# chenc10/distributed_TensorFlow_models

Measured on AMD Instinct MI355X. Metric: images/sec (whole node) ResNet-50 224×224 bf16 at 1/2/4/8 MI355X, higher is better.
Workload: dtype bf16; 1 GPU; model=resnet_v1_50, global_batch=256, per_gpu_batch=256, image_size=224, parallelism=dp1, device=cuda, grad_allreduce_dtype=fp32, deterministic=True, optimizer=momentum-sgd+wd

## Files before the change

csrc/kernels/conv_igemm.hip:

```cpp
#include "common.h"
#include <cstdio>

namespace dtm {


struct ConvNTArgs {
  const bf16_t* x;
  const bf16_t* w;
  bf16_t* y;
  float* stats;
  const float* bias;
  const float* in_scale;
  const float* in_shift;
  uint32_t x_bytes, w_bytes;
  int N, Hin, Win, C, K, R, S, P, Q;
  int stride, pad_h, pad_w;
  int Hv, Wv;
  int M;
  int Kg;
  int relu;
  FastDiv fd_PQ, fd_Q;
  const bf16_t* add_src;
  int add_stride;
  int add_H, add_W;
// ... 37 lines not shown
#undef DTM_GRP_LOAD
  }
  return t % gxy;
}

__device__ __forceinline__ void out_nhw(const ConvNTArgs& a, int m, int& n, int& h, int& w) {
  if (a.sp_tw) {
    const uint32_t t = (uint32_t)m >> 7, l = (uint32_t)m & 127u;
    const uint32_t nn = fdiv(t, a.fd_sp_img), rem = t - nn * (a.sp_th * a.sp_tw);
    const uint32_t th = fdiv(rem, a.fd_sp_tw), tw = rem - th * a.sp_tw;
    n = (int)nn;
    h = (int)(th * 8u + (l >> 4));
    w = (int)(tw * 16u + (l & 15u));
    return;
  }
  const uint32_t nn = fdiv((uint32_t)m, a.fd_PQ), rem = m - nn * (a.P * a.Q);
  const uint32_t i = fdiv(rem, a.fd_Q), j = rem - i * a.Q;
  n = (int)nn;
  h = (int)i * a.ostr + a.oa;
  w = (int)j * a.ostr + a.ob;
}
__device__ __forceinline__ int out_row(const ConvNTArgs& a, int m) {
  if (a.ostr == 1 && !a.sp_tw) return m;
  int n, h, w;
  out_nhw(a, m, n, h, w);
  return (n * a.OH + h) * a.OW + w;
}

__device__ __forceinline__ bool out_valid(const ConvNTArgs& a, int m) {
  if (!a.sp_tw) return true;
  int n, h, w;
  out_nhw(a, m, n, h, w);
  return h < a.P && w < a.Q;
}

template <bool RAWB>
__device__ __forceinline__ void epi_barrier() {
  if constexpr (RAWB) {
    asm volatile("s_waitcnt lgkmcnt(0)" ::: "memory");
    __builtin_amdgcn_s_barrier();
  } else {
    __syncthreads();
  }
}

template <int PT, int CT, bool RAWB, bool EXACT, bool SACC, int NT, bool SIDE = true, bool PRE = false, bool SPL = false,
          int EG = 4>
__device__ __forceinline__ void conv_nt_epi_tail(const ConvNTArgs& a, char* smem, int p0, int c0, int by,
                                                 float* ssum, float* ssq, const char* pre = nullptr,
                                                 const float* pre_ss = nullptr, float* aacc = nullptr) {
  constexpr int OROW = CT * 2 + 16;
  const int tid = threadIdx.x;
  epi_barrier<RAWB>();
  constexpr int CPR = CT / 8;
  constexpr int NIT = PT * CPR / NT;
  static_assert(NT % CPR == 0 && (PT * CPR) % NT == 0, "staged-store mapping");
  const int chn = tid % CPR;
  const int kc = c0 + chn * 8;
  const bool act = SIDE && a.act_x != nullptr;
  const bool bstats = !SACC && a.stats != nullptr;
  float sc[8], sh[8], sgx[8], sg[8];
#pragma unroll
  for (int e = 0; e < 8; ++e) { sc[e] = 1.f; sh[e] = 0.f; sgx[e] = 0.f; sg[e] = 0.f; }
  const bool amask = act && a.act_mask != nullptr;
  float sgr[8];
#pragma unroll
  for (int e = 0; e < 8; ++e) sgr[e] = 0.f;
  if (act && !amask && kc < a.K) {
#pragma unroll
    for (int e = 0; e < 8; ++e) {
      sc[e] = PRE ? pre_ss[chn * 8 + e] : a.act_ss[kc + e];
      sh[e] = PRE ? pre_ss[CT + chn * 8 + e] : a.act_ss[a.K + kc + e];
    }
  }
  constexpr int GRP = NIT < EG ? NIT : EG;
  static_assert(NIT % GRP == 0, "epilogue row groups");
  const bool side = SIDE && (a.add_src != nullptr || act);
#pragma unroll
  for (int g0 = 0; g0 < NIT; g0 += GRP) {
    uint4 pa[GRP], px[GRP], pr[GRP];
    uint32_t pm[GRP];
    bool ph[GRP];
#pragma unroll
    for (int j = 0; j < GRP; ++j) {
      pa[j] = px[j] = pr[j] = make_uint4(0, 0, 0, 0);
      pm[j] = 0u;
      ph[j] = false;
    }
    if (PRE && side) {
#pragma unroll
      for (int j = 0; j < GRP; ++j) {
        if (a.add_src) {
          pa[j] = *(const uint4*)(pre + (size_t)(g0 + j) * NT * 16 + tid * 16);
          ph[j] = true;
        }
        if (act) px[j] = *(const uint4*)(pre + (size_t)(NIT + g0 + j) * NT * 16 + tid * 16);
      }
    } else if (side) {
#pragma unroll
      for (int j = 0; j < GRP; ++j) {
        const int row = ((g0 + j) * NT + tid) / CPR;
        const int m = p0 + row;
        if (m < a.M && kc < a.K && out_valid(a, m)) {
          const size_t o = (size_t)out_row(a, m) * a.K + kc;
          if (a.add_src) {
            const bf16_t* src = a.add_src + o;
// ... 887 lines not shown
#pragma unroll
      for (int ii = 0; ii < 2; ++ii) {
        const int row = ni * 128 + wq * 32 + ii * 16 + fr;
        const short8 v = *(const short8*)(s + 2 * HALF + row * 128 + (((ks * 4 + fk) ^ (row & 7)) << 4));
        if (ni == 0) Wa[ks][ii] = v;
        else Wb[ks][ii] = v;
      }
  };
  auto mma = [&](int ni, int mi) {
#pragma unroll
    for (int ks = 0; ks < 2; ++ks)
#pragma unroll
      for (int ii = 0; ii < 2; ++ii)
#pragma unroll
        for (int jj = 0; jj < 4; ++jj)
          acc[ni][ii][mi][jj] = __builtin_amdgcn_mfma_f32_16x16x32_bf16(ni == 0 ? Wa[ks][ii] : Wb[ks][ii], P[ks][jj],
                                                                        acc[ni][ii][mi][jj], 0, 0, 0);
  };
  pp_mainloop(smem, BUF, nk, grp, issue, rd_p, rd_w, mma);
  __syncthreads();

#pragma unroll
  for (int ni = 0; ni < 2; ++ni)
#pragma unroll
    for (int ii = 0; ii < 2; ++ii) {
      const int kloc = ni * 128 + wq * 32 + ii * 16 + fk * 4;
      float bia[4] = {0.f, 0.f, 0.f, 0.f};
      if (a.bias && c0 + kloc < a.K) {
#pragma unroll
        for (int r = 0; r < 4; ++r) bia[r] = a.bias[c0 + kloc + r];
      }
#pragma unroll
      for (int mi = 0; mi < 2; ++mi)
#pragma unroll
        for (int jj = 0; jj < 4; ++jj) {
          const int mloc = mi * 128 + grp * 64 + jj * 16 + fr;
          float v[4];
#pragma unroll
          for (int r = 0; r < 4; ++r) {
            v[r] = acc[ni][ii][mi][jj][r] + bia[r];
            if (a.relu) v[r] = fmaxf(v[r], 0.f);
          }
          *(uint2*)(smem + mloc * OROW + kloc * 2) = make_uint2(pack2bf(v[0], v[1]), pack2bf(v[2], v[3]));
        }
    }
  conv_nt_epi_tail<PT, CT, false, false, false, 512, true, false, SPL>(a, smem, p0, c0, by, nullptr, nullptr);
}

template <int CT>
__device__ __forceinline__ void worker_row(float* red, const float* lo, const float* hi, float* row, int c0, int K) {
  constexpr int CPR = CT / 8, RPT = 256 / CPR;
  const int tid = threadIdx.x;
  __syncthreads();
#pragma unroll
  for (int e = 0; e < 8; ++e) { red[tid * 16 + e] = lo[e]; red[tid * 16 + 8 + e] = hi[e]; }
  __syncthreads();
  for (int h = RPT / 2; h >= 1; h >>= 1) {
    if (tid < h * CPR) {
#pragma unroll
      for (int e = 0; e < 16; ++e) red[tid * 16 + e] += red[(tid + h * CPR) * 16 + e];
    }
    __syncthreads();
  }
  const int kc = c0 + tid * 8;
  if (tid < CPR && kc < K) {
#pragma unroll
    for (int e = 0; e < 8; ++e) { row[kc + e] = red[tid * 16 + e]; row[K + kc + e] = red[tid * 16 + 8 + e]; }
  }
}

__device__ __forceinline__ void glds16(const void* gptr, const void* lds) {
  const uint32_t l = __builtin_amdgcn_readfirstlane((uint32_t)(uintptr_t)(const __attribute__((address_space(3))) void*)lds);
  asm volatile("s_mov_b32 m0, %1\n\ts_nop 0\n\tglobal_load_lds_dwordx4 %0, off" ::"v"(gptr), "s"(l) : "memory", "m0");
}

template <int PT, int CT, int NKT, bool PRO, bool STEM = false, int NBUF = 2, bool SIDE = true>
__global__ __launch_bounds__(256) void conv1x1_stream_kernel(ConvNTArgs a, int ntiles) {
  constexpr int WP = PT / 2, WC = CT / 2;
  constexpr int TP = WP / 16, TC = WC / 16;
  constexpr int AI = PT / 32, WI = CT / 32;
  constexpr int ABUF = NKT * PT * 128;
  constexpr int WBUF = NKT * CT * 128;
  constexpr int OROW = CT * 2 + 16;
  constexpr int STG = PT * OROW > 16384 ? PT * OROW : 16384;
  constexpr int NIT = PT * (CT / 8) / 256;
  constexpr int MAXC = 512;
  constexpr int OFF_A = WBUF, OFF_S = WBUF + NBUF * ABUF, OFF_P = OFF_S + STG;
  constexpr int NDMA = NKT * AI;
  static_assert(NBUF == 2 || NBUF == 3, "ring depth");
  static_assert(2 * NIT + NDMA <= 63, "vmcnt range");
  __shared__ __attribute__((aligned(16))) char smem[OFF_P + (PRO ? MAXC * 8 : 0)];
  typedef __attribute__((address_space(1))) const void gvoid;
  typedef __attribute__((address_space(3))) void lvoid;
  static_assert(NIT >= 1 && NIT <= 15, "vmcnt lower bound");

  const int tid = threadIdx.x, lane = tid & 63, wave = tid >> 6;
  const int nb = gridDim.x * gridDim.y;
  const int bid = xcd_remap(blockIdx.y * gridDim.x + blockIdx.x, nb);
  const int bx = bid % gridDim.x, by0 = bid / gridDim.x;
  const int c0 = bx * CT;
  const int lr = lane >> 3;
  const int ch = (lane & 7) ^ lr;
  const char* xg = (const char*)a.x;
  const char* wg = (const char*)a.w;
  const char* zg = (const char*)a.zero;
  float* s_scale = (float*)(smem + OFF_P);
  float* s_shift = s_scale + MAXC;
  if constexpr (PRO) {
    for (int c = tid; c < a.C; c += 256) { s_scale[c] = a.in_scale[c]; s_shift[c] = a.in_shift[c]; }
  }
#pragma unroll
  for (int kt = 0; kt < NKT; ++kt) {
#pragma unroll
    for (int j = 0; j < WI; ++j) {
      const int row = c0 + 8 * (wave + 4 * j) + lr;
      const int k = kt * 64 + ch * 8;
      const bool v = (row < a.K) & (k < a.Kg);
      const char* src = wg + (size_t)(uint32_t)((row * a.Kg + k) * 2);
      __builtin_amdgcn_global_load_lds((gvoid*)(v ? src : zg), (lvoid*)(smem + kt * CT * 128 + (wave + 4 * j) * 1024),
                                       16, 0, 0);
    }
  }
  const char* srcs[NKT * AI];
  auto issue = [&](int t, int buf) {
    char* base = smem + OFF_A + buf * ABUF;
    uint32_t pix[AI];
    if constexpr (STEM) {
#pragma unroll
      for (int j = 0; j < AI; ++j) {
        const int m = t * PT + 8 * (wave + 4 * j) + lr;
        const uint32_t mm = m < a.M ? (uint32_t)m : 0u;
        const uint32_t n = fdiv(mm, a.fd_PQ), rem = mm - n * (a.P * a.Q);
        const uint32_t p = fdiv(rem, a.fd_Q), q = rem - p * a.Q;
        pix[j] = ((n * a.Hin + p * a.stride) * a.Win + q * a.stride) * 8u;
      }
    }
#pragma unroll
    for (int kt = 0; kt < NKT; ++kt) {
      const int k = kt * 64 + ch * 8;
#pragma unroll
      for (int j = 0; j < AI; ++j) {
        const int m = t * PT + 8 * (wave + 4 * j) + lr;
        const bool v = (m < a.M) & (k < a.Kg);
        const char* src = STEM ? xg + (size_t)(pix[j] + (uint32_t)((k >> 5) * a.Win * 8 + (k & 31) * 2))
                               : xg + (size_t)(uint32_t)(m * a.pix_bytes + k * 2);
        srcs[kt * AI + j] = v ? src : zg;
        glds16(srcs[kt * AI + j], base + kt * PT * 128 + (wave + 4 * j) * 1024);
      }
    }
  };
  auto transform = [&](int t, int buf) {
    char* base = smem + OFF_A + buf * ABUF;
#pragma unroll
    for (int kt = 0; kt < NKT; ++kt) {
      const int k = kt * 64 + ch * 8;
      if (k < a.Kg) {
        const float4 s0 = *(const float4*)(s_scale + k), s1 = *(const float4*)(s_scale + k + 4);
        const float4 h0 = *(const float4*)(s_shift + k), h1 = *(const float4*)(s_shift + k + 4);
        const float sc[8] = {s0.x, s0.y, s0.z, s0.w, s1.x, s1.y, s1.z, s1.w};
        const float sh[8] = {h0.x, h0.y, h0.z, h0.w, h1.x, h1.y, h1.z, h1.w};
#pragma unroll
        for (int j = 0; j < AI; ++j) {
          const int m = t * PT + 8 * (wave + 4 * j) + lr;
          if (m < a.M) {
            uint4* pp = (uint4*)(base + kt * PT * 128 + (wave + 4 * j) * 1024 + lane * 16);
            const uint4 q = *pp;
            uint32_t u[4] = {q.x, q.y, q.z, q.w};
#pragma unroll
            for (int e = 0; e < 4; ++e) {
              const float lo = fmaxf(fmaf(lo_bf(u[e]), sc[2 * e], sh[2 * e]), 0.f);
              const float hi = fmaxf(fmaf(hi_bf(u[e]), sc[2 * e + 1], sh[2 * e + 1]), 0.f);
              u[e] = pack2bf(lo, hi);
            }
            *pp = make_uint4(u[0], u[1], u[2], u[3]);
          }
        }
      }
    }
  };

  const int wp = wave % 2, wc = wave / 2;
  const int fr = lane & 15, fk = lane >> 4;
  float ssum[8], ssq[8], aacc[24];
#pragma unroll
  for (int e = 0; e < 8; ++e) { ssum[e] = 0.f; ssq[e] = 0.f; }
#pragma unroll
  for (int e = 0; e < 24; ++e) aacc[e] = 0.f;
  int t = by0;
  const int gy = gridDim.y;
  if (t < ntiles) issue(t, 0);
  if (NBUF == 3 && t + gy < ntiles) issue(t + gy, 1);
  asm volatile("s_waitcnt vmcnt(0)" ::: "memory");
  __syncthreads();
  int buf = 0;
  for (int it = 0; t < ntiles; ++it, t += gy) {
    if constexpr (NBUF == 2) {
      if (it > 0) asm volatile("s_waitcnt vmcnt(%0)" ::"n"(NIT) : "memory");
    } else if (it >= 2) {
      if (t + gy < ntiles) asm volatile("s_waitcnt vmcnt(%0)" ::"n"(2 * NIT + NDMA) : "memory");
      else asm volatile("s_waitcnt vmcnt(%0)" ::"n"(2 * NIT) : "memory");
    }
    if constexpr (PRO) transform(t, buf);
    asm volatile("s_waitcnt lgkmcnt(0)" ::: "memory");
    __builtin_amdgcn_s_barrier();
    if constexpr (NBUF == 2) {
      if (t + gy < ntiles) issue(t + gy, buf ^ 1);
    } else {
      if (t + 2 * gy < ntiles) issue(t + 2 * gy, buf == 0 ? 2 : buf - 1);
    }
    f32x4 acc[TC][TP];
#pragma unroll
    for (int i = 0; i < TC; ++i)
#pragma unroll
      for (int j = 0; j < TP; ++j) acc[i][j] = (f32x4){0.f, 0.f, 0.f, 0.f};
    const char* abase = smem + OFF_A + buf * ABUF;
#pragma unroll
    for (int kt = 0; kt < NKT; ++kt) {
#pragma unroll
      for (int ks = 0; ks < 2; ++ks) {
        short8 bf[TP], af[TC];
        const int chn = ks * 4 + fk;
#pragma unroll
        for (int j = 0; j < TP; ++j) {
          const int row = wp * WP + j * 16 + fr;
          bf[j] = *(const short8*)(abase + kt * PT * 128 + row * 128 + ((chn ^ (row & 7)) << 4));
        }
#pragma unroll
        for (int i = 0; i < TC; ++i) {
          const int row = wc * WC + i * 16 + fr;
          af[i] = *(const short8*)(smem + kt * CT * 128 + row * 128 + ((chn ^ (row & 7)) << 4));
        }
#pragma unroll
        for (int i = 0; i < TC; ++i)
#pragma unroll
          for (int j = 0; j < TP; ++j)
            acc[i][j] = __builtin_amdgcn_mfma_f32_16x16x32_bf16(af[i], bf[j], acc[i][j], 0, 0, 0);
      }
    }
    conv_nt_epilogue<PT, CT, WP, WC, 1, true, true, true, true, 256, SIDE>(a, acc, smem + OFF_S, t * PT, c0, t, ssum,
                                                                           ssq, nullptr, nullptr, aacc);
#pragma unroll
    for (int i = 0; i < NKT * AI; ++i) asm volatile("" ::"v"(srcs[i]));
    buf = buf + 1 == NBUF ? 0 : buf + 1;
  }
  asm volatile("s_waitcnt vmcnt(0)" ::: "memory");
  if (a.stats) worker_row<CT>((float*)(smem + OFF_S), ssum, ssq, a.stats + (size_t)by0 * (2 * a.K), c0, a.K);
  if (SIDE && a.act_x && a.act_sums) {
    const int rw = a.act_r ? 4 : 2;
    float* row = a.act_sums + (size_t)by0 * (rw * a.K);
    worker_row<CT>((float*)(smem + OFF_S), aacc, aacc + 8, row, c0, a.K);
    if (a.act_r) worker_row<CT>((float*)(smem + OFF_S), aacc + 16, aacc + 8, row + 2 * a.K, c0, a.K);
  }
}

template <int CIN>
__device__ __forceinline__ int dsw(int p, int c) {
  return CIN == 64 ? (c ^ ((p >> 1) & 7)) : (c ^ ((p >> 2) & 3));
}

template <int CIN, int CT, bool SIDE>
__global__ __launch_bounds__(256) void conv3x3_direct_kernel(ConvNTArgs a, int ntiles) {
  constexpr int TH = 8, TW = 16, PT = TH * TW, HH = TH + 2, HW = TW + 2;
  constexpr int CPP = CIN / 8;
  constexpr int HCH = HH * HW * CPP;
  constexpr int NDMA = (HCH + 255) / 256;
  constexpr int OROW = CT * 2 + 16;
  constexpr int HDMA = NDMA * 256 * 16;
  constexpr int HBUF = HDMA > PT * OROW ? HDMA : PT * OROW;
  static_assert(3 * HBUF >= 256 * 16 * 4, "worker_row's reduction table fits in the ring");
  constexpr int WBUF = 9 * CT * CIN * 2;
  constexpr int NIT = PT * (CT / 8) / 256;
  constexpr int TC = CT / 16, TP = 2;
  constexpr int SD = SIDE ? 2 * NIT : 0;
  constexpr int SBUF = SIDE ? 2 * NIT * 4096 + 2 * CT * 4 : 0;
  static_assert(2 * NIT + SD + NDMA <= 63, "vmcnt range");
  __shared__ __attribute__((aligned(16))) char smem[WBUF + 3 * HBUF + SBUF];
  char* sside = smem + WBUF + 3 * HBUF;
  float* s_ss = (float*)(sside + 2 * NIT * 4096);

  const int tid = threadIdx.x, lane = tid & 63, wave = tid >> 6;
  const int nb = gridDim.x * gridDim.y;
  const int bid = xcd_remap(blockIdx.y * gridDim.x + blockIdx.x, nb);
  const int bx = bid % gridDim.x, by0 = bid / gridDim.x;
  const int c0 = bx * CT;
  const char* xg = (const char*)a.x;
  const char* zg = (const char*)a.zero;
  const int tiles_w = a.sp_tw, tiles_img = a.sp_th * a.sp_tw;

  if constexpr (SIDE) {
    for (int j = tid; j < 2 * CT; j += 256) {
      const int ch = j % CT, k = c0 + ch;
      s_ss[j] = (a.act_x && k < a.K) ? a.act_ss[(j / CT) * a.K + k] : (j < CT ? 1.f : 0.f);
// ... 988 lines not shown
  const int n = flip_tiles(f);
  for (int t = blockIdx.x; t < n; t += gridDim.x) flip_tile(f, t, lds);
}

}

using namespace dtm;

struct ConvDesc {
  int N, H, W, C, K, R, S, P, Q, stride, pad_h, pad_w;
  int pix_bytes;
  int dec;
};

static const bf16_t* zero_chunk() {
  static void* z = nullptr;
  if (!z) {
    if (hipMalloc(&z, 4096) != hipSuccess) return nullptr;
    hipMemset(z, 0, 4096);
    hipDeviceSynchronize();
  }
  return (const bf16_t*)z;
}
const void* dtm_zero_chunk() { return zero_chunk(); }

template <int PT, int CT, int NWP, int NS, int UD, bool SPL = false, int NTH = 512>
static void launch_w8(const ConvNTArgs& a, hipStream_t st) {
  dim3 grid((a.K + CT - 1) / CT, (a.M + PT - 1) / PT, a.ngrp > 1 ? a.ngrp : 1);
  hipLaunchKernelGGL((conv_nt_w8_kernel<PT, CT, NWP, NS, UD, SPL, NTH>), grid, dim3(NTH), 0, st, a);
}

template <int UD, bool SPL = false>
static void launch_pp(const ConvNTArgs& a, hipStream_t st) {
  dim3 grid((a.K + 255) / 256, (a.M + 255) / 256, a.ngrp > 1 ? a.ngrp : 1);
  hipLaunchKernelGGL((conv_nt_pp_kernel<UD, SPL>), grid, dim3(512), 0, st, a);
}

template <int PT, int CT, int NS, int UD, int NWP = 2, bool SPL = false>
static void launch_pipe(const ConvNTArgs& a, hipStream_t st) {
  dim3 grid((a.K + CT - 1) / CT, (a.M + PT - 1) / PT, a.ngrp > 1 ? a.ngrp : 1);
  if (SPL) hipLaunchKernelGGL((conv_nt_pipe_kernel<PT, CT, NS, UD, false, NWP, true>), grid, dim3(256), 0, st, a);
  else if (a.in_scale) hipLaunchKernelGGL((conv_nt_pipe_kernel<PT, CT, NS, UD, true, NWP>), grid, dim3(256), 0, st, a);
  else hipLaunchKernelGGL((conv_nt_pipe_kernel<PT, CT, NS, UD, false, NWP>), grid, dim3(256), 0, st, a);
}

static int device_cus() { return dtm_compute_cus(); }

static bf16_t* dump_chunk() {
  static void* z = nullptr;
  if (!z && hipMalloc(&z, 4096) != hipSuccess) return nullptr;
  return (bf16_t*)z;
}

template <int PT, int CT, int NKT, bool PRO, bool STEM = false, int NBUF = 2, bool SIDE = true>
static int stream_workers_k(const ConvNTArgs& a) {
  static int occ = 0;
  if (!occ) {
    if (hipOccupancyMaxActiveBlocksPerMultiprocessor(&occ, conv1x1_stream_kernel<PT, CT, NKT, PRO, STEM, NBUF, SIDE>,
                                                     256, 0) !=
            hipSuccess || occ <= 0)
      occ = 1;
  }
  const int ctiles = (a.K + CT - 1) / CT;
  const int ntiles = (a.M + PT - 1) / PT;
  int workers = (occ * device_cus() + ctiles - 1) / ctiles;
  if (workers > ntiles) workers = ntiles;
  if (workers < 1) workers = 1;
  return workers;
}

template <int PT, int CT, int NKT, bool PRO, bool STEM = false, int NBUF = 2, bool SIDE = true>
static void launch_stream_k(const ConvNTArgs& a, hipStream_t st) {
  const int ctiles = (a.K + CT - 1) / CT;
  const int ntiles = (a.M + PT - 1) / PT;
  hipLaunchKernelGGL((conv1x1_stream_kernel<PT, CT, NKT, PRO, STEM, NBUF, SIDE>),
                     dim3(ctiles, stream_workers_k<PT, CT, NKT, PRO, STEM, NBUF, SIDE>(a)), dim3(256), 0, st, a, ntiles);
}

static bool stem_stream_ok(const ConvNTArgs& a) {
  return a.pix_bytes == 8 && a.C == 32 && a.S == 1 && a.pad_h == 0 && a.pad_w == 0 && a.Kg == a.R * 32 &&
         a.Kg <= 256 && a.K % 64 == 0 && !a.in_scale && !a.bias && !a.relu && a.ostr == 1;
}

template <int CT, int NKT>
static void launch_stream(const ConvNTArgs& a, hipStream_t st) {
  const bool side = a.add_src || a.act_x;
  if (a.in_scale) {
    if (side) launch_stream_k<64, CT, NKT, true, false, 2, true>(a, st);
    else launch_stream_k<64, CT, NKT, true, false, 2, false>(a, st);
  } else if (side) launch_stream_k<64, CT, NKT, false, false, 2, true>(a, st);
  else launch_stream_k<64, CT, NKT, false, false, 2, false>(a, st);
}
template <int CT, int NKT>
static int stream_workers(const ConvNTArgs& a) {
  const bool side = a.add_src || a.act_x;
  if (a.in_scale) return side ? stream_workers_k<64, CT, NKT, true, false, 2, true>(a)
                              : stream_workers_k<64, CT, NKT, true, false, 2, false>(a);
  if (side) return stream_workers_k<64, CT, NKT, false, false, 2, true>(a);
  return stream_workers_k<64, CT, NKT, false, false, 2, false>(a);
}

static int g_stem_stream = 1;
DTM_API void dtm_conv_set_stem_stream(int on) { g_stem_stream = on; }
static int stream_rows(const ConvNTArgs& a, int id) {
  if (id == 33) return g_stem_stream == 2 ? stream_workers_k<64, 64, 4, false, true, 2, false>(a)
                                          : stream_workers_k<64, 64, 4, false, true, 3, false>(a);
  const bool k1 = a.Kg <= 64;
  if (id == 30) {
    return k1 ? stream_workers<128, 1>(a) : stream_workers<128, 2>(a);
  }
  return k1 ? stream_workers<64, 1>(a) : stream_workers<64, 2>(a);
}

static bool stream_ok(const ConvNTArgs& a) {
  return !a.bias && !a.relu && a.R == 1 && a.S == 1 && a.stride == 1 && a.pad_h == 0 && a.pad_w == 0 && a.Hv == a.Hin && a.Wv == a.Win &&
         a.P == a.Hin && a.Q == a.Win && a.Kg % 64 == 0 && a.Kg <= 128 && a.K % 8 == 0 &&
         (!a.in_scale || a.C <= 512) && a.dump != nullptr && a.ostr == 1;
}

template <int PT, int CT, int WP, int WC, int UD, int NBUF = 2, bool SPL = false, int LBW = 0, int EG = 4>
static void launch_nt(const ConvNTArgs& a, hipStream_t st) {
  dim3 grid((a.K + CT - 1) / CT, (a.M + PT - 1) / PT, a.ngrp > 1 ? a.ngrp : 1);
  hipLaunchKernelGGL((conv_nt_kernel<PT, CT, WP, WC, UD, NBUF, SPL, LBW, EG>), grid, dim3(256), 0, st, a);
}
static int g_act_occ = getenv("DTM_ACT_OCC") ? atoi(getenv("DTM_ACT_OCC")) : 2;
DTM_API void dtm_conv_set_act_occ(int v) { g_act_occ = v; }
static int g_nt_occ = getenv("DTM_NT_OCC") ? atoi(getenv("DTM_NT_OCC")) : 2;
DTM_API void dtm_conv_set_nt_occ(int v) { g_nt_occ = v; }
template <int PT, int CT, int UD>
static void launch_nt_act(const ConvNTArgs& a, hipStream_t st) {
  const bool side = (a.K & 7) == 0 && (a.add_src != nullptr || a.act_x != nullptr);
  const int v = side ? g_act_occ : (a.stats ? 0 : g_nt_occ);
  if (v == 1) launch_nt<PT, CT, 32, 64, UD, 1, false, 0, 2>(a, st);
  else if (v == 2) launch_nt<PT, CT, 32, 64, UD, 1, false, 4, 4>(a, st);
  else if (v == 3) launch_nt<PT, CT, 32, 64, UD, 1, false, 4, 2>(a, st);
  else launch_nt<PT, CT, 32, 64, UD, 1>(a, st);
}

static int g_direct3 = 1;
DTM_API void dtm_conv_set_direct3(int on) { g_direct3 = on; }
static bool direct_ok(const ConvNTArgs& a) {
  return a.R == 3 && a.S == 3 && a.stride == 1 && a.Hv == a.Hin && a.Wv == a.Win && (a.C == 32 || a.C == 64) &&
         a.K % 32 == 0 && !a.in_scale && !a.bias && !a.relu && a.pix_bytes == a.C * 2 && a.ostr == 1 &&
         a.pad_h <= 2 && a.pad_w <= 2 && !a.act_mask && !a.act_r && (!a.add_src || a.add_stride == 1);
}
static void direct_setup(ConvNTArgs& a) {
  a.sp_tw = (a.Q + 15) / 16;
  a.sp_th = (a.P + 7) / 8;
  a.fd_sp_img = make_fastdiv(a.sp_th * a.sp_tw);
  a.fd_sp_tw = make_fastdiv(a.sp_tw);
  a.M = a.N * a.sp_th * a.sp_tw * 128;
}
template <int CIN, int CT, bool SIDE>
static int direct_workers_k(const ConvNTArgs& a) {
  static int occ = 0;
  if (!occ) {
    if (hipOccupancyMaxActiveBlocksPerMultiprocessor(&occ, conv3x3_direct_kernel<CIN, CT, SIDE>, 256, 0) != hipSuccess ||
        occ <= 0)
// ... 78 lines not shown
    if (a.K <= 32 && g_k32_tile) id = 32;
    else if (a.K <= 64) id = 26;
    else if (a.K <= 128) id = 21;
  }
  if (id == -1 && g_kwide && a.K > 64 && a.K % 128 != 0 && (a.K % 128) <= 64 && a.K % 8 == 0)
    id = a.in_scale ? 3 : ((g_policy2 && a.M >= 16384 && (a.M <= 65536 || a.M >= 262144)) ? 24 : 26);
  if (id == -1 && !a.in_scale && a.Kg >= 1024) {
    id = 21;
    if (g_policy2 && (long)((a.M + 127) / 128) * ((a.K + 127) / 128) <= device_cus()) id = 26;
  }
  if (id == -1 && !a.in_scale && a.K <= 64 && a.R * a.S > 1 && a.K % 64 == 0) id = 26;
  if (id < 0) id = a.K <= 64 ? g_k64_tile : ((a.M <= 16384 && a.Kg >= 2048) ? 0 : 4);
  if ((id == 21 || id == 24 || id == 26 || id == 32) && a.in_scale && a.C > 512) id = 0;
  if (id == 21 || id == 26) return {id, 128, 2};
  if (id == 24) return {id, 256, 2};
  if (id == 32) return {id, 256, 4};
  if ((id == 40 || id == 41) && a.in_scale) id = 0;
  if (id == 40 && g_tile_pp && g_tile_env != 40) id = 41;
  if (id == 41 && a.K % 8) id = 40;
  if (id == 40 || id == 41) return {id, 256, 2};
  if (id == 30 || id == 31) {
    if (stream_ok(a)) return {id, 64, 2};
    id = a.K <= 64 ? 3 : 4;
  }
  if (id == 3) return {id, 128, 4};
  if (id == 4) return {id, 64, 2};
  return {0, 128, 2};
}

static void dispatch_split(const ConvNTArgs& a, const TileCfg& t, hipStream_t st) {
  if (t.id == 3) launch_nt<128, 64, 32, 64, 1, 1, true>(a, st);
  else if (t.id == 4) launch_nt<64, 128, 32, 64, 1, 1, true>(a, st);
  else if (t.id == 21) launch_pipe<128, 128, 2, 1, 2, true>(a, st);
  else if (t.id == 24) launch_pipe<256, 64, 2, 1, 2, true>(a, st);
  else if (t.id == 26) launch_pipe<128, 64, 2, 1, 2, true>(a, st);
  else if (t.id == 32) launch_pipe<256, 32, 2, 1, 4, true>(a, st);
  else if (t.id == 40) launch_w8<256, 256, 2, 2, 1, true>(a, st);
  else if (t.id == 41) launch_pp<1, true>(a, st);
  else launch_nt<128, 128, 64, 64, 1, 2, true>(a, st);
}

template <int UD>
static void dispatch_ud(const ConvNTArgs& a, const TileCfg& t, hipStream_t st) {
  if (UD == 1 && a.nsplit > 0) dispatch_split(a, t, st);
  else if (t.id == 3) launch_nt_act<128, 64, UD>(a, st);
  else if (t.id == 4) launch_nt_act<64, 128, UD>(a, st);
  else if (t.id == 30 && UD == 1) {
    if (a.Kg <= 64) launch_stream<128, 1>(a, st);
    else launch_stream<128, 2>(a, st);
  } else if (t.id == 60 && UD == 1) {
    launch_direct(a, st);
  } else if (t.id == 33 && UD == 1) {
    if (g_stem_stream == 2) launch_stream_k<64, 64, 4, false, true, 2, false>(a, st);
    else launch_stream_k<64, 64, 4, false, true, 3, false>(a, st);
  } else if (t.id == 31 && UD == 1) {
    if (a.Kg <= 64) launch_stream<64, 1>(a, st);
    else launch_stream<64, 2>(a, st);
  } else if (t.id == 21) launch_pipe<128, 128, 2, UD>(a, st);
  else if (t.id == 24) launch_pipe<256, 64, 2, UD>(a, st);
  else if (t.id == 26) launch_pipe<128, 64, 2, UD>(a, st);
  else if (t.id == 32) launch_pipe<256, 32, 2, UD, 4>(a, st);
  else if (t.id == 40) launch_w8<256, 256, 2, 2, UD>(a, st);
  else if (t.id == 41) launch_pp<UD>(a, st);
  else launch_nt<128, 128, 64, 64, UD>(a, st);
}

DTM_API void dtm_conv_set_tile(int id) { g_tile_env = id; }

static void dispatch_nt(const ConvNTArgs& a, int ud, const TileCfg& t, hipStream_t st) {
  if (ud == 1) dispatch_ud<1>(a, t, st);
  else dispatch_ud<2>(a, t, st);
}

DTM_API int dtm_get_deterministic();

static int g_split_tile = 1;
DTM_API void dtm_conv_set_split_tile(int on) { g_split_tile = on; }

static int conv_fwd_impl(const void* x, const void* w, void* y, bool stats, const float* bias, const float* in_scale,
                         const float* in_shift, int relu, const ConvDesc* d, hipStream_t stream, float** rows_ws,
                         int* nrows, const ConvNTArgs::Split* split = nullptr, int nsplit = 0) {
  if (!dtm_device_ok()) return -9;
  if (d->C % 8 || d->K % 4) return -1;
  ConvNTArgs a;
  a.x = (const bf16_t*)x; a.w = (const bf16_t*)w; a.y = (bf16_t*)y;
  a.ngrp = 0;
  a.nsplit = 0;
  a.stats = nullptr; a.bias = bias; a.in_scale = in_scale; a.in_shift = in_shift;
  a.add_src = nullptr; a.act_x = nullptr; a.act_ss = nullptr; a.act_sums = nullptr;
  a.act_mask = nullptr; a.act_r = nullptr;
  a.add_stride = 1; a.add_H = a.add_W = 0;
  a.act_unscaled = 0;
  a.zero = zero_chunk();
  a.dump = dump_chunk();
  a.pix_bytes = d->pix_bytes > 0 ? d->pix_bytes : d->C * 2;
  size_t xb = (size_t)d->N * d->H * d->W * a.pix_bytes, wb = (size_t)d->K * d->R * d->S * d->C * 2;
  if (xb >= (1ull << 31) || wb >= (1ull << 31)) return -2;
  a.x_bytes = (uint32_t)xb; a.w_bytes = (uint32_t)wb;
  a.N = d->N; a.Hin = d->H; a.Win = d->W; a.C = d->C; a.K = d->K; a.R = d->R; a.S = d->S;
  a.P = d->P; a.Q = d->Q; a.stride = d->stride; a.pad_h = d->pad_h; a.pad_w = d->pad_w;
  a.Hv = d->H; a.Wv = d->W;
  a.M = d->N * d->P * d->Q; a.Kg = d->R * d->S * d->C; a.relu = relu;
  a.fd_PQ = make_fastdiv(d->P * d->Q); a.fd_Q = make_fastdiv(d->Q);
  a.ostr = 1; a.oa = a.ob = 0; a.OH = a.P; a.OW = a.Q;
  a.sp_tw = a.sp_th = 0;
  if (nsplit > 0) {
// ... 457 lines not shown
```

distributed_tensorflow_models_amd/ops/_lib.py:

```python
import ctypes
import os

import torch

_HERE = os.path.dirname(os.path.dirname(os.path.abspath(__file__)))
LIB_PATH = os.environ.get("DTM_KERNELS_SO") or os.path.join(_HERE, "_native", "libdtm_kernels.so")

_lib = None


class ConvDesc(ctypes.Structure):
    _fields_ = [(n, ctypes.c_int) for n in
                ("N", "H", "W", "C", "K", "R", "S", "P", "Q", "stride", "pad_h", "pad_w", "pix_bytes", "dec")]


class PoolArgs(ctypes.Structure):
    _fields_ = [(n, ctypes.c_int) for n in
                ("N", "H", "W", "C", "P", "Q", "KH", "KW", "SH", "SW", "PH", "PW")]


_P = ctypes.c_void_p
_I = ctypes.c_int
_L = ctypes.c_long
_F = ctypes.c_float
_D = ctypes.c_double

_SIGS = {
    "dtm_conv_fwd": (_I, [_P, _P, _P, _P, _P, _P, _P, _I, ctypes.POINTER(ConvDesc), _P]),
    "dtm_act_fwd": (_I, [_P, _P, _L, _I, _F, _I, _P]),
    "dtm_prep_params_bytes": (_I, []),
    "dtm_jpeg_desc_bytes": (_I, []),
    "dtm_jpeg_decode_gpu": (_I, [_P, _P, _I, _I, _L, _P, _P, _P]),
    "dtm_jpeg_huff_desc_bytes": (_I, []),
    "dtm_jpeg_huff_gpu": (_I, [_P, _P, _P, _I, _P, _P, _P]),
    "dtm_jpeg_set_huff": (None, [_I, _I]),
    "dtm_imagenet_prep": (_I, [_P, _P, _P, _P, _P, _I, _I, _I, _P]),
    "dtm_act_bwd": (_I, [_P, _P, _P, _L, _I, _F, _I, _P]),
    "dtm_instnorm_fwd": (_I, [_P, _P, _P, _P, _P, _I, _I, _I, _F, _I, _I, _P]),
    "dtm_instnorm_bwd": (_I, [_P, _P, _P, _P, _P, _P, _I, _I, _I, _I, _P]),
    "dtm_reflect_pad": (_I, [_P, _P, _I, _I, _I, _I, _I, _I, _I, _I, _I, _P]),
    "dtm_reflect_pad_bwd": (_I, [_P, _P, _I, _I, _I, _I, _I, _I, _I, _I, _I, _P]),
    "dtm_conv_dgrad": (_I, [_P, _P, _P, ctypes.POINTER(ConvDesc), _P]),
    "dtm_conv_dgrad_ex": (_I, [_P, _P, _P, ctypes.POINTER(ConvDesc), _P, _I, _P, _P, _P, _I, _P]),
    "dtm_conv_dgrad_bnout": (_I, [_P, _P, _P, ctypes.POINTER(ConvDesc), _P, _I, _P, _P, _P, _P, _P]),
    "dtm_conv1x1_bnbwd": (_I, [_P, _P, _P, _P, _P, _F, _P, _P, _P, _P, _P, _I, _P, _P, _P, _P, _L, _I, _I, _P]),
    "dtm_conv_wgrad_bnbwd": (_I, [_P, _P, _P, _P, _P, _P, _F, _P, _P, _P, ctypes.POINTER(ConvDesc), _I, _P]),
    "dtm_conv_wgrad": (_I, [_P, _P, _P, _P, _P, ctypes.POINTER(ConvDesc), _I, _P]),
    "dtm_conv_wgrad_multi": (_I, [_P, _P, _P, _P, _I, ctypes.POINTER(ConvDesc), _I, _P]),
    "dtm_conv_set_policy2": (None, [_I]),
    "dtm_set_grid_cpt": (None, [_I]),
    "dtm_conv_set_k32": (None, [_I]),
    "dtm_conv_set_stem_stream": (None, [_I]),
    "dtm_ws_set_side_stream": (None, [_I, _P]),
    "dtm_device_check": (_I, []),
    "dtm_conv_set_direct3": (None, [_I]),
    "dtm_conv_set_dec_group": (None, [_I]),
    "dtm_cat_desc_bytes": (_I, []),
    "dtm_cat_bn_apply": (_I, [_P, _I, _P, _L, _I, _P]),
    "dtm_cat_bn_apply_bwd": (_I, [_P, _I, _P, _P, _L, _I, _P]),
    "dtm_weight_flip_transpose": (None, [_P, _P, _I, _I, _I, _I, _P]),
    "dtm_weight_flip_transpose_batched": (None, [_P, _I, _P]),
    "dtm_weight_flip_transpose_dec": (None, [_P, _P, _I, _I, _I, _I, _I, _I, _I, _P]),
    "dtm_flip_desc_bytes": (_I, []),
    "dtm_bn_stats": (None, [_P, _P, _L, _I, _P]),
    "dtm_col_sums": (_I, [_P, _P, _L, _I, _P]),
    "dtm_bn_stats_bwd": (_I, [_P, _P, _P, _P, _L, _I, _P]),
    "dtm_bn_finalize": (None, [_P, _P, _P, _P, _P, _P, _I, _F, _F, _F, _I, _I, _P]),
    "dtm_bn_inference_params": (None, [_P, _P, _P, _P, _P, _I, _F, _P]),
    "dtm_bn_apply": (None, [_P, _P, _P, _P, _P, _L, _I, _I, _I, _P]),
    "dtm_bn_apply2": (_I, [_P, _P, _P, _P, _P, _P, _L, _I, _I, _I, _P]),
    "dtm_maxpool_bnrelu_fwd": (_I, [_P, _P, _P, _P, ctypes.POINTER(PoolArgs), _P]),
    "dtm_maxpool_bnrelu_bwd": (_I, [_P, _P, _P, _P, _P, _P, ctypes.POINTER(PoolArgs), _I, _P]),
    "dtm_conv_set_tile": (None, [_I]),
    "dtm_conv_set_wgrad_tile": (None, [_I, _I]),
    "dtm_loss_combine": (_I, [_P, _I, _I, _P, _P, _P]),
    "dtm_scale_rows_pad": (_I, [_P, _I, _P, _I, _P, _I, _I, _I, _P]),
    "dtm_conv_set_wgrad_k64": (None, [_I]),
    "dtm_pool_set_k3s2": (None, [_I]),
    "dtm_conv_fwd_bn": (_I, [_P, _P, _P, _P, _P, _P, _P, _P, _P, _P, _F, _F, _F, _I, _I, ctypes.POINTER(ConvDesc), _P]),
    "dtm_stats_combine_fin": (_I, [_P, _P, _P, _P, _P, _F, _P, _P, _P, _L, _I, _I, _P]),
    "dtm_stats_combine_fin_ld": (_I, [_P, _P, _P, _P, _P, _F, _P, _P, _P, _L, _I, _I, _I, _P]),
    "dtm_bn_apply_res_strided": (_I, [_P, _P, _P, _P, _P, _I, _I, _I, _I, _I, _I, _I, _I, _P]),
    "dtm_bn_bwd_reduce": (None, [_P, _P, _P, _P, _P, _L, _I, _I, _P]),
    "dtm_bn_bwd_apply": (None, [_P, _P, _P, _P, _P, _P, _P, _L, _I, _I, _I, _P]),
    "dtm_bn_param_grad": (None, [_P, _P, _P, _I, _P]),
    "dtm_maxpool_fwd": (None, [_P, _P, _P, ctypes.POINTER(PoolArgs), _P]),
    "dtm_maxpool_bwd": (None, [_P, _P, _P, ctypes.POINTER(PoolArgs), _P]),
    "dtm_maxpool_bwd_ld": (_I, [_P, _I, _P, _P, ctypes.POINTER(PoolArgs), _P]),
    "dtm_avgpool_fwd": (None, [_P, _P, ctypes.POINTER(PoolArgs), _I, _P]),
    "dtm_avgpool_bwd": (None, [_P, _P, ctypes.POINTER(PoolArgs), _I, _P]),
    "dtm_avgpool_bwd_acc": (_I, [_P, _P, ctypes.POINTER(PoolArgs), _I, _P]),
    "dtm_global_avg_fwd": (None, [_P, _P, _I, _I, _I, _P]),
    "dtm_global_avg_bwd": (None, [_P, _P, _I, _I, _I, _P]),
    "dtm_global_avg_fwd_bf16": (None, [_P, _P, _I, _I, _I, _P]),
    "dtm_global_avg_bwd_bf16": (None, [_P, _P, _I, _I, _I, _P]),
    "dtm_softmax_xent": (None, [_P, _I, _P, _P, _P, _I, _I, _F, _F, _P, _I, _P]),
    "dtm_opt_chunk_size": (_I, []),
    "dtm_opt_tensor_bytes": (_I, []),
    "dtm_opt_chunk_bytes": (_I, []),
# ... 214 lines not shown
```

distributed_tensorflow_models_amd/ops/features.py:

```python
import contextlib
import os

FEATURES = {
    "fused_bn": ("conv -> BatchNorm as one lazily applied pair: statistics in the conv epilogue, the BN-apply + ReLU "
                 "folded into the consumer (models/layers.py)", "profiles/r1_resnet50_b256_fused_v1_summary.txt (vs r1_torch_eager_baseline_probe.log)"),
    "sibling_group": ("one backward for the sibling 1x1 conv+BNs reading one input (Inception branch heads, a ResNet "
                      "projection unit's shortcut + conv1)", "profiles/ab/r3_ab_sibling_resnet.log, r4_ab_sibling_inception.log"),
    "sibling_fwd": ("Inception mixed blocks: the branch-head 1x1 conv+BNs as ONE conv over their concatenated weights "
                    "+ one grouped BN finalize", "profiles/ab/r4_ab_sibfwd_inception.log"),
    "sibling_combine": ("the sibling members' BN stats-combines as one grouped launch",
                        "profiles/ab/r4_ab_knobs_inception.log"),
    "act_handoff": ("conv consumers of one activation hand the masked input gradient on (the last one's act epilogue "
                    "adds it)", "profiles/ab/r4_ab_sibling_inception.log"),
    "bnout_fuse": ("the block-output BN-apply backward inside the consuming conv's dgrad epilogue",
                   "profiles/ab/r2_ab_bnout.log, r3_ab_dgrp_bnst.log"),
    "bwd1x1_fuse": ("one-pass backward of ResNet's 64->256 expansion 1x1 conv+BN", "profiles/ab/r2_ab_bwd1x1.log"),
    "stem_wgrad_fuse": ("the stem's BN backward inside its wgrad operand staging", "profiles/ab/r2_ab_stem_wgrad_bn.log"),
    "cat_multi": ("an Inception block's concat BN-apply as one multi-part launch", "profiles/ab/r2_ab_cat_multi_inception.log"),
    "pool_commute": ("Inception pool branches as conv -> pool -> BN (the pool over the conv's output channels)",
                     "profiles/ab/r2_ab_pool_commute_inception.log"),
    "wgrad_stream": ("conv+BN weight gradients on a second HIP stream, concurrent with the dgrad chain "
                     "(TrainStep(wgrad_stream=...) overrides per model)", "profiles/ab/r3_ab_wgrad_side_stream.log"),
    "pool_tail": ("Inception's aux-head pool gradient added in place into the Mixed_6e-output gradient the main path "
                  "returned (no separate add over the 17x17x768 map)", "profiles/ab/r5_ab_pool_tail.log"),
    "bsp_compact": ("dead-tap conv weights get a compact all-reduce bucket holding their live window only",
                    "tests/test_distributed.py test_bsp_dead_tap_gradients_left_out_of_the_allreduce"),
}

ROUTES_GRADIENTS = ("fused_bn", "sibling_group", "sibling_fwd", "sibling_combine", "act_handoff", "bnout_fuse",
                    "bwd1x1_fuse", "stem_wgrad_fuse", "cat_multi", "pool_commute", "wgrad_stream", "bsp_compact")

_override = {}


def _disabled_env():
    v = os.environ.get("DTM_DISABLE", "")
    return {n.strip() for n in v.split(",") if n.strip()}


def on(name):
    if name not in FEATURES:
        raise KeyError("unknown feature %r (ops/features.py)" % name)
    if name in _override:
        return _override[name]
    return name not in _disabled_env()


def check_env():
    bad = sorted(_disabled_env() - set(FEATURES))
    if bad:
        raise ValueError("DTM_DISABLE names unknown features %s (known: %s)" % (bad, ", ".join(sorted(FEATURES))))


@contextlib.contextmanager
def override(**kw):
    for k in kw:
        if k not in FEATURES:
            raise KeyError("unknown feature %r" % k)
    saved = {k: _override.get(k) for k in kw}
    _override.update({k: bool(v) for k, v in kw.items()})
    try:
        yield
    finally:
        for k, v in saved.items():
            if v is None:
                _override.pop(k, None)
            else:
                _override[k] = v


# ... 3 lines not shown
```

distributed_tensorflow_models_amd/ops/fused.py:

```python
import ctypes

import torch

from . import _lib, features
from .geometry import conv_geom
from .lazy import LazyBN, Subsampled, as_tensor
from .nn import _accum_param_grad, _check, _notify, dgrad_decomposable, grad_target, weight_bf16, weight_flipped


class ZeroArena:

    def __init__(self, floats=1 << 22):
        self.floats = floats
        self.buf = None
        self.off = 0
        self.high = 0
        self.active = False

    def begin_step(self, device):
        if self.buf is None or self.buf.device != device:
            self.buf = torch.zeros(self.floats, device=device, dtype=torch.float32)
            self.high = 0
        elif self.high:
            self.buf[:self.high].zero_()
# ... 448 lines not shown
                dx = dx + dx2
                sx = sx + sx2
                if sr is not None:
                    sr = sr + sr2
            info.g = info.sums = None
            dres = None if not ctx.res_mode else dx
        else:
            dx = torch.empty_like(x)
            dres = None if not ctx.res_mode else (dx if alias else torch.empty_like(x))
            sx = arena.zeros((4, C), x.device)
            sr = arena.zeros((4, C), x.device) if ctx.res_mode == 2 else None
            mode = 3 if mask is not None else (1 if ctx.relu else 0)
            _check(L.dtm_bn_apply_bwd(_lib.ptr(dy.contiguous()), _lib.ptr(y), _lib.ptr(mask), _lib.ptr(x),
                                      _lib.ptr(ss), _lib.ptr(res), _lib.ptr(rss), _lib.ptr(dx), _lib.ptr(dres),
                                      _lib.ptr(sx), _lib.ptr(sr), M, C, mode, ctx.res_mode, ctx.unscaled,
                                      _lib.stream_ptr()), "bn_apply_bwd")
        st = ctx.res_stride
        if ctx.res_slot is not None:
            last, buf, bst = _slot_take(ctx.res_slot)
            if not last:
                _slot_stash(ctx.res_slot, dres, st)
                dres = None
            elif buf is not None or st > 1:
                dres = _unstride(ctx.res_slot, dres, st)
                if buf is not None:
                    dres = dres + _unstride(ctx.res_slot, buf, bst)
        elif st > 1:
            full = torch.zeros(ctx.res_shape, device=dres.device, dtype=dres.dtype)
            full[:, ::st, ::st, :] = dres
            dres = full
        return dx, sx, dres, sr, None, None, None, None


class _StemConvBNFn(torch.autograd.Function):

    @staticmethod
    def forward(ctx, x, w, gamma, beta, geom, bn, pad):
        L = _lib.lib()
        s = _lib.stream_ptr()
        N, H, W, C = x.shape
        K, R, S, _ = w.shape
        st, P, Q = geom.stride, geom.P, geom.Q
        Hp = max(H + 2 * pad, st * (P - 1) + R)
        Wp = max(W + 2 * pad, st * (Q - 1) + 8)
        Wp += Wp % 2
        if x.dtype in (torch.float32, torch.bfloat16) and x.is_contiguous():
            xp = torch.empty((N, Hp, Wp, 4), device=x.device, dtype=torch.bfloat16)
            _check(L.dtm_stem_pack(_lib.ptr(x), 0 if x.dtype == torch.float32 else 1, _lib.ptr(xp), N, H, W, C, Hp,
                                   Wp, pad, s), "stem_pack")
        else:
            xp = torch.nn.functional.pad(x.to(torch.bfloat16), (0, 4 - C, pad, Wp - W - pad, pad, Hp - H - pad))
        wv = torch.zeros((K, R, 8, 4), device=x.device, dtype=torch.bfloat16)
        wv[:, :, :S, :C] = weight_bf16(w)
        d = _lib.ConvDesc(N, Hp, Wp, 32, K, R, 1, P, Q, st, 0, 0, 8)
        y = torch.empty((N, P, Q, K), device=x.device, dtype=torch.bfloat16)
        ss = None
        if bn is not None:
            ss = torch.empty((4, K), device=x.device, dtype=torch.float32)
            ctx.count = float(N * P * Q)
            _check(L.dtm_conv_fwd_bn(_lib.ptr(xp), _lib.ptr(wv), _lib.ptr(y), None, None, _lib.ptr(gamma),
                                     _lib.ptr(beta), _lib.ptr(bn.moving_mean), _lib.ptr(bn.moving_variance),
                                     _lib.ptr(ss), ctx.count, float(bn.eps), float(bn.decay), 1, int(bn.bessel),
                                     ctypes.byref(d), s), "stem_conv_fwd_bn")
        else:
            _check(L.dtm_conv_fwd(_lib.ptr(xp), _lib.ptr(wv), _lib.ptr(y), None, None, None, None, 0,
                                  ctypes.byref(d), s), "stem_conv_fwd")
        ctx.d = (N, Hp, Wp, K, R, S, C, P, Q, st)
        ctx.save_for_backward(xp, w, y, ss, gamma, beta)
        if ss is None:
            return y
        return y, ss

    @staticmethod
    def backward(ctx, dy, dss=None):
        L = _lib.lib()
        s = _lib.stream_ptr()
        xp, w, y, ss, gamma, beta = ctx.saved_tensors
        N, Hp, Wp, K, R, S, C, P, Q, st = ctx.d
        dy = dy.contiguous()
        dgamma = dbeta = None
        if (ss is not None and dss is not None and ctx.needs_input_grad[1] and features.on("stem_wgrad_fuse")):
            gmg = grad_target(gamma) if gamma is not None else None
            bmg = grad_target(beta) if beta is not None else None
            dgamma = torch.zeros(K, device=dy.device) if (gamma is not None and gmg is None) else None
            dbeta = torch.zeros(K, device=dy.device) if (beta is not None and bmg is None) else None
            d = _lib.ConvDesc(N, Hp, Wp, 32, K, R, 1, P, Q, st, 0, 0, 8)
            tv = torch.zeros((K, R, 8, 4), device=dy.device, dtype=torch.float32)
            _check(L.dtm_conv_wgrad_bnbwd(_lib.ptr(xp), _lib.ptr(dy), _lib.ptr(y), _lib.ptr(dss.contiguous()),
                                          _lib.ptr(ss), _lib.ptr(gamma), ctx.count,
                                          _lib.ptr(gmg if gmg is not None else dgamma),
                                          _lib.ptr(bmg if bmg is not None else dbeta), _lib.ptr(tv), ctypes.byref(d),
                                          _lib.wgrad_cus("stem"), s), "stem_conv_wgrad_bnbwd")
            for p, m in ((gamma, gmg), (beta, bmg)):
                if m is not None:
                    _notify(p)
            dw = _accum_param_grad(w, tv[:, :, :S, :C])
            return None, dw, dgamma, dbeta, None, None, None
        if ss is not None and dss is not None:
            gmg = grad_target(gamma) if gamma is not None else None
            bmg = grad_target(beta) if beta is not None else None
            if gamma is not None and gmg is None:
                dgamma = torch.zeros(K, device=dy.device)
            if beta is not None and bmg is None:
                dbeta = torch.zeros(K, device=dy.device)
            comb = torch.empty_like(dy)
            _check(L.dtm_stats_combine_fin(_lib.ptr(dy), _lib.ptr(y), _lib.ptr(dss.contiguous()), _lib.ptr(ss),
# ... 553 lines not shown
```

Measured before the change: 14740 images/sec.

## Trim stem k-loop to real columns and run stem stream with 8 waves

The stem forward's persistent stream kernel now stops its reduction loop and operand loads at the packed rows' real reduction width (R*32 of NKT*64 columns), skipping MFMAs and DMA on zero padding. It also gains an 8-wave-per-block variant (512 threads, two waves per SIMD) for the 64x64 tiles with a 3-slot ring. Extra waves only issue loads and MFMAs, while the epilogue is limited to the first 256 threads. The change adds wave-dependent vmcnt waits and register/LDS pressure, which could lower occupancy or break the wait accounting.

```diff
diff --git a/csrc/kernels/conv_igemm.hip b/csrc/kernels/conv_igemm.hip
--- a/csrc/kernels/conv_igemm.hip
+++ b/csrc/kernels/conv_igemm.hip
@@ -113,6 +113,7 @@
   constexpr int OROW = CT * 2 + 16;
   const int tid = threadIdx.x;
   epi_barrier<RAWB>();
+  if (SACC && !SIDE && tid >= NT) return;
   constexpr int CPR = CT / 8;
   constexpr int NIT = PT * CPR / NT;
   static_assert(NT % CPR == 0 && (PT * CPR) % NT == 0, "staged-store mapping");
@@ -1106,8 +1107,10 @@
   constexpr int CPR = CT / 8, RPT = 256 / CPR;
   const int tid = threadIdx.x;
   __syncthreads();
-#pragma unroll
-  for (int e = 0; e < 8; ++e) { red[tid * 16 + e] = lo[e]; red[tid * 16 + 8 + e] = hi[e]; }
+  if (tid < 256) {
+#pragma unroll
+    for (int e = 0; e < 8; ++e) { red[tid * 16 + e] = lo[e]; red[tid * 16 + 8 + e] = hi[e]; }
+  }
   __syncthreads();
   for (int h = RPT / 2; h >= 1; h >>= 1) {
     if (tid < h * CPR) {
@@ -1128,16 +1131,21 @@
   asm volatile("s_mov_b32 m0, %1\n\ts_nop 0\n\tglobal_load_lds_dwordx4 %0, off" ::"v"(gptr), "s"(l) : "memory", "m0");
 }
 
-template <int PT, int CT, int NKT, bool PRO, bool STEM = false, int NBUF = 2, bool SIDE = true>
-__global__ __launch_bounds__(256) void conv1x1_stream_kernel(ConvNTArgs a, int ntiles) {
-  constexpr int WP = PT / 2, WC = CT / 2;
+template <int PT, int CT, int NKT, bool PRO, bool STEM = false, int NBUF = 2, bool SIDE = true, int NTH = 256>
+__global__ __launch_bounds__(NTH) void conv1x1_stream_kernel(ConvNTArgs a, int ntiles, int klim) {
+  constexpr int NW = NTH / 64;
+  constexpr int WP = PT / 2, WC = CT / (NW / 2);
   constexpr int TP = WP / 16, TC = WC / 16;
-  constexpr int AI = PT / 32, WI = CT / 32;
+  constexpr int AI = PT / (8 * NW), WI = CT / (8 * NW);
+  static_assert(NW == 4 || NW == 8, "4 or 8 waves");
+  static_assert(AI >= 1 && WI >= 1 && TC >= 1, "tile too small for the wave count");
   constexpr int ABUF = NKT * PT * 128;
   constexpr int WBUF = NKT * CT * 128;
   constexpr int OROW = CT * 2 + 16;
   constexpr int STG = PT * OROW > 16384 ? PT * OROW : 16384;
-  constexpr int NIT = PT * (CT / 8) / 256;
+  constexpr int NTT = 256;
+  static_assert(NTH == NTT || (!SIDE && NBUF == 3), "the 8-wave form: no side inputs, 3-slot ring");
+  constexpr int NIT = PT * (CT / 8) / NTT;
   constexpr int MAXC = 512;
   constexpr int OFF_A = WBUF, OFF_S = WBUF + NBUF * ABUF, OFF_P = OFF_S + STG;
   constexpr int NDMA = NKT * AI;
@@ -1161,17 +1169,17 @@
   float* s_scale = (float*)(smem + OFF_P);
   float* s_shift = s_scale + MAXC;
   if constexpr (PRO) {
-    for (int c = tid; c < a.C; c += 256) { s_scale[c] = a.in_scale[c]; s_shift[c] = a.in_shift[c]; }
+    for (int c = tid; c < a.C; c += NTH) { s_scale[c] = a.in_scale[c]; s_shift[c] = a.in_shift[c]; }
   }
 #pragma unroll
   for (int kt = 0; kt < NKT; ++kt) {
 #pragma unroll
     for (int j = 0; j < WI; ++j) {
-      const int row = c0 + 8 * (wave + 4 * j) + lr;
+      const int row = c0 + 8 * (wave + NW * j) + lr;
       const int k = kt * 64 + ch * 8;
       const bool v = (row < a.K) & (k < a.Kg);
       const char* src = wg + (size_t)(uint32_t)((row * a.Kg + k) * 2);
-      __builtin_amdgcn_global_load_lds((gvoid*)(v ? src : zg), (lvoid*)(smem + kt * CT * 128 + (wave + 4 * j) * 1024),
+      __builtin_amdgcn_global_load_lds((gvoid*)(v ? src : zg), (lvoid*)(smem + kt * CT * 128 + (wave + NW * j) * 1024),
                                        16, 0, 0);
     }
   }
@@ -1182,7 +1190,7 @@
     if constexpr (STEM) {
 #pragma unroll
       for (int j = 0; j < AI; ++j) {
-        const int m = t * PT + 8 * (wave + 4 * j) + lr;
+        const int m = t * PT + 8 * (wave + NW * j) + lr;
         const uint32_t mm = m < a.M ? (uint32_t)m : 0u;
         const uint32_t n = fdiv(mm, a.fd_PQ), rem = mm - n * (a.P * a.Q);
         const uint32_t p = fdiv(rem, a.fd_Q), q = rem - p * a.Q;
@@ -1194,12 +1202,13 @@
       const int k = kt * 64 + ch * 8;
 #pragma unroll
       for (int j = 0; j < AI; ++j) {
-        const int m = t * PT + 8 * (wave + 4 * j) + lr;
+        const int m = t * PT + 8 * (wave + NW * j) + lr;
         const bool v = (m < a.M) & (k < a.Kg);
         const char* src = STEM ? xg + (size_t)(pix[j] + (uint32_t)((k >> 5) * a.Win * 8 + (k & 31) * 2))
                                : xg + (size_t)(uint32_t)(m * a.pix_bytes + k * 2);
         srcs[kt * AI + j] = v ? src : zg;
-        glds16(srcs[kt * AI + j], base + kt * PT * 128 + (wave + 4 * j) * 1024);
+        if (!STEM || k < klim || kt * 64 >= klim)
+          glds16(srcs[kt * AI + j], base + kt * PT * 128 + (wave + NW * j) * 1024);
       }
     }
   };
@@ -1215,9 +1224,9 @@
         const float sh[8] = {h0.x, h0.y, h0.z, h0.w, h1.x, h1.y, h1.z, h1.w};
 #pragma unroll
         for (int j = 0; j < AI; ++j) {
-          const int m = t * PT + 8 * (wave + 4 * j) + lr;
+          const int m = t * PT + 8 * (wave + NW * j) + lr;
           if (m < a.M) {
-            uint4* pp = (uint4*)(base + kt * PT * 128 + (wave + 4 * j) * 1024 + lane * 16);
+            uint4* pp = (uint4*)(base + kt * PT * 128 + (wave + NW * j) * 1024 + lane * 16);
             const uint4 q = *pp;
             uint32_t u[4] = {q.x, q.y, q.z, q.w};
 #pragma unroll
@@ -1251,7 +1260,10 @@
     if constexpr (NBUF == 2) {
       if (it > 0) asm volatile("s_waitcnt vmcnt(%0)" ::"n"(NIT) : "memory");
     } else if (it >= 2) {
-      if (t + gy < ntiles) asm volatile("s_waitcnt vmcnt(%0)" ::"n"(2 * NIT + NDMA) : "memory");
+      if (NTH > NTT && wave >= NTT / 64) {
+        if (t + gy < ntiles) asm volatile("s_waitcnt vmcnt(%0)" ::"n"(NDMA) : "memory");
+        else asm volatile("s_waitcnt vmcnt(0)" ::: "memory");
+      } else if (t + gy < ntiles) asm volatile("s_waitcnt vmcnt(%0)" ::"n"(2 * NIT + NDMA) : "memory");
       else asm volatile("s_waitcnt vmcnt(%0)" ::"n"(2 * NIT) : "memory");
     }
     if constexpr (PRO) transform(t, buf);
@@ -1272,6 +1284,7 @@
     for (int kt = 0; kt < NKT; ++kt) {
 #pragma unroll
       for (int ks = 0; ks < 2; ++ks) {
+        if (STEM && kt * 64 + ks * 32 >= klim) continue;
         short8 bf[TP], af[TC];
         const int chn = ks * 4 + fk;
 #pragma unroll
@@ -1291,7 +1304,7 @@
             acc[i][j] = __builtin_amdgcn_mfma_f32_16x16x32_bf16(af[i], bf[j], acc[i][j], 0, 0, 0);
       }
     }
-    conv_nt_epilogue<PT, CT, WP, WC, 1, true, true, true, true, 256, SIDE>(a, acc, smem + OFF_S, t * PT, c0, t, ssum,
+    conv_nt_epilogue<PT, CT, WP, WC, 1, true, true, true, true, NTT, SIDE>(a, acc, smem + OFF_S, t * PT, c0, t, ssum,
                                                                            ssq, nullptr, nullptr, aacc);
 #pragma unroll
     for (int i = 0; i < NKT * AI; ++i) asm volatile("" ::"v"(srcs[i]));
@@ -2386,12 +2399,16 @@
   return (bf16_t*)z;
 }
 
-template <int PT, int CT, int NKT, bool PRO, bool STEM = false, int NBUF = 2, bool SIDE = true>
+static int g_stem_ktrim = 1;
+DTM_API void dtm_conv_set_stem_ktrim(int on) { g_stem_ktrim = on; }
+
+template <int PT, int CT, int NKT, bool PRO, bool STEM = false, int NBUF = 2, bool SIDE = true, int NTH = 256>
 static int stream_workers_k(const ConvNTArgs& a) {
   static int occ = 0;
   if (!occ) {
-    if (hipOccupancyMaxActiveBlocksPerMultiprocessor(&occ, conv1x1_stream_kernel<PT, CT, NKT, PRO, STEM, NBUF, SIDE>,
-                                                     256, 0) !=
+    if (hipOccupancyMaxActiveBlocksPerMultiprocessor(&occ,
+                                                     conv1x1_stream_kernel<PT, CT, NKT, PRO, STEM, NBUF, SIDE, NTH>,
+                                                     NTH, 0) !=
             hipSuccess || occ <= 0)
       occ = 1;
   }
@@ -2403,12 +2420,13 @@
   return workers;
 }
 
-template <int PT, int CT, int NKT, bool PRO, bool STEM = false, int NBUF = 2, bool SIDE = true>
+template <int PT, int CT, int NKT, bool PRO, bool STEM = false, int NBUF = 2, bool SIDE = true, int NTH = 256>
 static void launch_stream_k(const ConvNTArgs& a, hipStream_t st) {
   const int ctiles = (a.K + CT - 1) / CT;
   const int ntiles = (a.M + PT - 1) / PT;
-  hipLaunchKernelGGL((conv1x1_stream_kernel<PT, CT, NKT, PRO, STEM, NBUF, SIDE>),
-                     dim3(ctiles, stream_workers_k<PT, CT, NKT, PRO, STEM, NBUF, SIDE>(a)), dim3(256), 0, st, a, ntiles);
+  hipLaunchKernelGGL((conv1x1_stream_kernel<PT, CT, NKT, PRO, STEM, NBUF, SIDE, NTH>),
+                     dim3(ctiles, stream_workers_k<PT, CT, NKT, PRO, STEM, NBUF, SIDE, NTH>(a)), dim3(NTH), 0, st, a, ntiles,
+                     STEM && g_stem_ktrim ? a.Kg : NKT * 64);
 }
 
 static bool stem_stream_ok(const ConvNTArgs& a) {
@@ -2434,10 +2452,13 @@
   return stream_workers_k<64, CT, NKT, false, false, 2, false>(a);
 }
 
+static int g_stem_w8 = 1;
+DTM_API void dtm_conv_set_stem_w8(int on) { g_stem_w8 = on; }
 static int g_stem_stream = 1;
 DTM_API void dtm_conv_set_stem_stream(int on) { g_stem_stream = on; }
 static int stream_rows(const ConvNTArgs& a, int id) {
   if (id == 33) return g_stem_stream == 2 ? stream_workers_k<64, 64, 4, false, true, 2, false>(a)
+                       : g_stem_w8        ? stream_workers_k<64, 64, 4, false, true, 3, false, 512>(a)
                                           : stream_workers_k<64, 64, 4, false, true, 3, false>(a);
   const bool k1 = a.Kg <= 64;
   if (id == 30) {
@@ -2622,6 +2643,7 @@
     launch_direct(a, st);
   } else if (t.id == 33 && UD == 1) {
     if (g_stem_stream == 2) launch_stream_k<64, 64, 4, false, true, 2, false>(a, st);
+    else if (g_stem_w8) launch_stream_k<64, 64, 4, false, true, 3, false, 512>(a, st);
     else launch_stream_k<64, 64, 4, false, true, 3, false>(a, st);
   } else if (t.id == 31 && UD == 1) {
     if (a.Kg <= 64) launch_stream<64, 1>(a, st);
diff --git a/distributed_tensorflow_models_amd/ops/_lib.py b/distributed_tensorflow_models_amd/ops/_lib.py
--- a/distributed_tensorflow_models_amd/ops/_lib.py
+++ b/distributed_tensorflow_models_amd/ops/_lib.py
@@ -45,6 +45,8 @@
     "dtm_conv_dgrad_bnout": (_I, [_P, _P, _P, ctypes.POINTER(ConvDesc), _P, _I, _P, _P, _P, _P, _P]),
     "dtm_conv1x1_bnbwd": (_I, [_P, _P, _P, _P, _P, _F, _P, _P, _P, _P, _P, _I, _P, _P, _P, _P, _L, _I, _I, _P]),
     "dtm_conv_wgrad_bnbwd": (_I, [_P, _P, _P, _P, _P, _P, _F, _P, _P, _P, ctypes.POINTER(ConvDesc), _I, _P]),
+    "dtm_conv_set_stem_ktrim": (None, [_I]),
+    "dtm_conv_set_stem_w8": (None, [_I]),
     "dtm_conv_wgrad": (_I, [_P, _P, _P, _P, _P, ctypes.POINTER(ConvDesc), _I, _P]),
     "dtm_conv_wgrad_multi": (_I, [_P, _P, _P, _P, _I, ctypes.POINTER(ConvDesc), _I, _P]),
     "dtm_conv_set_policy2": (None, [_I]),
diff --git a/distributed_tensorflow_models_amd/ops/features.py b/distributed_tensorflow_models_amd/ops/features.py
--- a/distributed_tensorflow_models_amd/ops/features.py
+++ b/distributed_tensorflow_models_amd/ops/features.py
@@ -16,6 +16,10 @@
                    "profiles/ab/r2_ab_bnout.log, r3_ab_dgrp_bnst.log"),
     "bwd1x1_fuse": ("one-pass backward of ResNet's 64->256 expansion 1x1 conv+BN", "profiles/ab/r2_ab_bwd1x1.log"),
     "stem_wgrad_fuse": ("the stem's BN backward inside its wgrad operand staging", "profiles/ab/r2_ab_stem_wgrad_bn.log"),
+    "stem_ktrim": ("the stem forward's k-loop stops at the packed rows' R * 32 real reduction columns",
+                   "profiles/ab/stem_chain_ab.log"),
+    "stem_w8": ("the stem forward's persistent stream with 8 waves per block (two per SIMD) on the same 64-pixel tiles",
+                "profiles/ab/stem_chain_ab.log"),
     "cat_multi": ("an Inception block's concat BN-apply as one multi-part launch", "profiles/ab/r2_ab_cat_multi_inception.log"),
     "pool_commute": ("Inception pool branches as conv -> pool -> BN (the pool over the conv's output channels)",
                      "profiles/ab/r2_ab_pool_commute_inception.log"),
diff --git a/distributed_tensorflow_models_amd/ops/fused.py b/distributed_tensorflow_models_amd/ops/fused.py
--- a/distributed_tensorflow_models_amd/ops/fused.py
+++ b/distributed_tensorflow_models_amd/ops/fused.py
@@ -524,6 +524,8 @@
             xp = torch.nn.functional.pad(x.to(torch.bfloat16), (0, 4 - C, pad, Wp - W - pad, pad, Hp - H - pad))
         wv = torch.zeros((K, R, 8, 4), device=x.device, dtype=torch.bfloat16)
         wv[:, :, :S, :C] = weight_bf16(w)
+        L.dtm_conv_set_stem_ktrim(int(features.on("stem_ktrim")))
+        L.dtm_conv_set_stem_w8(int(features.on("stem_w8")))
         d = _lib.ConvDesc(N, Hp, Wp, 32, K, R, 1, P, Q, st, 0, 0, 8)
         y = torch.empty((N, P, Q, K), device=x.device, dtype=torch.bfloat16)
         ss = None
```

Result: no change. 14700 images/sec (-0.3%).
